# CelestineAngla/BundleAdjustment.jl

Hardware: AMD Instinct MI355X
Metric: LM iterations/sec on BAL venice-1778 (synthetic BAL-shaped), plus Jacobian Mnnz/sec (higher is better)
Workload: dtype f64; 1 GPU; venice-1778 shape: ncams=1778 npnts=993923 nobs=5001946, seed 20261004, lm.jl variant, LDL/None, facto_type f64, fixed 83 iterations, perm AMD; parallelism=points sharded over 1 rank(s), cameras replicated

## Files before the change

### bundleadjustment.jl_amd/csrc/ba_dense_ldl.hip

```cpp
#include "ba_internal.h"

#include <algorithm>
#include <atomic>
#include <cmath>
#include <cstdio>
#include <cstdlib>

namespace {

template <typename T>
struct RT;
template <>
struct RT<double> {
  typedef double v4 __attribute__((ext_vector_type(4)));
  typedef double v2 __attribute__((ext_vector_type(2)));
  static __device__ inline v4 mfma(double a, double b, v4 c) { return __builtin_amdgcn_mfma_f64_16x16x4f64(a, b, c, 0, 0, 0); }
  static __device__ inline int row(int lane, int reg) { return (lane >> 4) + 4 * reg; }
};
template <>
struct RT<float> {
  typedef float v4 __attribute__((ext_vector_type(4)));
  typedef float v2 __attribute__((ext_vector_type(2)));
  static __device__ inline v4 mfma(float a, float b, v4 c) { return __builtin_amdgcn_mfma_f32_16x16x4f32(a, b, c, 0, 0, 0); }
  static __device__ inline int row(int lane, int reg) { return 4 * (lane >> 4) + reg; }
// ... 246 lines not shown
#pragma unroll
      for (int i = m + 1; i < 16; i++) sacc[i] += col[i] * y;
      xj[m * XDL + c] = xv;
      Linv_k[(o + m) * NB + o + c] = xv;
      __builtin_amdgcn_sched_barrier(0);
#pragma unroll
      for (int i = m + 2; i < 16; i++) col[i] = nxt[i];
    }
  };
  auto inv_finalize = [&](int I, int J) {
    d4 acc;
#pragma unroll
    for (int g = 0; g < 4; g++) acc[g] = a[(16 * J + fr) * LDA2 + 16 * I + RT<T>::row(lane, g)];
    d4 out = {0, 0, 0, 0};
#pragma unroll
    for (int g = 0; g < 4; g++) out = RT<T>::mfma(xd[(I * 16 + fr) * XDL + RT<T>::row(lane, g)], acc[g], out);
#pragma unroll
    for (int g = 0; g < 4; g++) {
      a[(16 * J + fr) * LDA2 + 16 * I + RT<T>::row(lane, g)] = -out[g];
      Linv_k[(16 * I + RT<T>::row(lane, g)) * NB + 16 * J + fr] = -out[g];
    }
  };
  auto inv_update = [&](int I, int J, int K) {
    d4 acc = {0, 0, 0, 0};
    if (K > J) {
#pragma unroll
      for (int g = 0; g < 4; g++) acc[g] = a[(16 * J + fr) * LDA2 + 16 * I + RT<T>::row(lane, g)];
    }
#pragma unroll
    for (int kk = 0; kk < 4; kk++) {
      const int k = 16 * K + 4 * kk + fk;
      const T af = a[(16 * I + fr) * LDA2 + k] * dinv[k];
      const T *bp = (K == J) ? xd + (J * 16 + fk) * XDL + fr : a + (16 * J + fr) * LDA2 + 16 * K + fk;
      const int bstep = (K == J) ? 4 * XDL : 4;
      acc = RT<T>::mfma(af, bp[kk * bstep], acc);
    }
#pragma unroll
    for (int g = 0; g < 4; g++) a[(16 * J + fr) * LDA2 + 16 * I + RT<T>::row(lane, g)] = acc[g];
  };
  constexpr int NWK = NW - 1;
  auto do_pivots = [&](int jb) {
    if constexpr (sizeof(T) == 8) pivots_mfma(jb);
    else pivots(jb);
  };
  if (wv == 0) do_pivots(0);
  __syncthreads();
  STAMP(1)
  row_solves(0);
  if (wv == 3 && lane < 16) inv16(0);
  __syncthreads();
  STAMP(2)
  if constexpr (NW == 8) {
    constexpr int CAP = 3 * NWK - 1;
    const int u = (wv == 4) ? 6 : (wv < 4 ? wv - 1 : wv - 2);
    const int h = (wv == 2) ? 0 : (wv == 6) ? 1 : (wv == 4) ? 2 : (wv == 5) ? 3 : (wv == 7) ? 4 : -1;
    auto f_task = [&](int s, int t) {
      int ii = 0;
      while ((ii + 1) * (ii + 2) / 2 <= t) ii++;
      const int jj = t - ii * (ii + 1) / 2;
      block_update(s, s + 2 + ii, s + 2 + jj);
    };
    for (int s = 0; s < 7; s++) {
      const int nX = s, nC = 6 - s, nU = s * (7 - s), nF = (6 - s) * (7 - s) / 2;
      const int nfix = nX + nC + nU, nP = nfix + nF < CAP ? nfix + nF : (nfix > CAP ? nfix : CAP);
      unsigned long long c0 = 0;
      if (stamps) c0 = __builtin_amdgcn_s_memtime();
      if (wv == 0) {
        block_update(s, s + 1, s + 1);
        __builtin_amdgcn_fence(__ATOMIC_RELEASE, "wavefront");
        __builtin_amdgcn_wave_barrier();
        __builtin_amdgcn_fence(__ATOMIC_ACQUIRE, "wavefront");
        do_pivots(s + 1);
      } else {
        for (int r = 0; r < 3 + (nfix + NWK - 1) / NWK; r++) {
          const int t = r < 2 ? NWK * r + u : 2 * NWK + (NWK - 1) * (r - 2) + u;
          if ((r >= 2 && u == NWK - 1) || t >= nP) continue;
          if (t < nX) {
            inv_finalize(s, t);
          } else if (t < nX + nC) {
            block_update(s, s + 2 + (t - nX), s + 1);
          } else if (t < nfix) {
            const int e = t - nX - nC;
            inv_update(s + 1 + e % (7 - s), e / (7 - s), s - 1);
          } else {
            f_task(s, t - nfix);
          }
        }
      }
      if (stamps && lane == 0) stamps[6 + s * 8 + wv] = __builtin_amdgcn_s_memtime() - c0;
      __syncthreads();
      STAMP(1)
      if (stamps) c0 = __builtin_amdgcn_s_memtime();
      row_solves(s + 1);
      if (wv == 3 && lane < 16) inv16(s + 1);
      if (h >= 0) {
        const int nA = (s + 1) + (nfix + nF - nP);
        for (int t = h; t < nA; t += 5) {
          if (t <= s) inv_update(s + 1, t, s);
          else f_task(s, nP - nfix + (t - (s + 1)));
        }
      }
      if (stamps && lane == 0) stamps[62 + s * 8 + wv] = __builtin_amdgcn_s_memtime() - c0;
      __syncthreads();
      STAMP(2)
    }
  } else {
    for (int jb = 0; jb < 7; jb++) {
      for (int t = wv; t < 7; t += NW) {
        if (t < 7 - jb) block_update(jb, jb + 1 + t, jb + 1);
        else inv_finalize(jb, t - (7 - jb));
      }
      __syncthreads();
      STAMP(3)
      unsigned long long c0 = 0;
      if (stamps) c0 = __builtin_amdgcn_s_memtime();
      if (wv == 0) {
        do_pivots(jb + 1);
      } else {
        const int mb = 6 - jb, nblk = mb * (mb + 1) / 2, ninv = (7 - jb) * (jb + 1);
        for (int t = wv - 1; t < nblk + ninv; t += NWK) {
          if (t < nblk) {
            int ii = 0;
            while ((ii + 1) * (ii + 2) / 2 <= t) ii++;
            const int jj = t - ii * (ii + 1) / 2;
            block_update(jb, jb + 2 + ii, jb + 2 + jj);
          } else {
            const int e = t - nblk, J = e / (7 - jb), I = jb + 1 + e % (7 - jb);
            inv_update(I, J, jb);
          }
        }
      }
      if (stamps && lane == 0) stamps[6 + jb * 8 + wv] = __builtin_amdgcn_s_memtime() - c0;
      __syncthreads();
      STAMP(1)
      row_solves(jb + 1);
      if (wv == 3 && lane < 16) inv16(jb + 1);
      __syncthreads();
      STAMP(2)
    }
  }
  for (int J = wv; J < 7; J += NW) inv_finalize(7, J);
  if (tid < NB) D_k[tid] = dd[tid];
  STAMP(4)
  if (stamps && tid == 0)
    for (int q = 0; q < 6; q++) stamps[q] = tacc[q];
#undef STAMP
}

template <typename T>
__global__ __launch_bounds__(DIAG_THREADS) void k_ldl_diag(T *__restrict__ Skk, T *__restrict__ Linv_k,
                                                   T *__restrict__ D_k, int *__restrict__ flag,
                                                   unsigned long long *__restrict__ stamps,
                                                   const int *__restrict__ wait_ready, int clear_flag) {
  extern __shared__ __attribute__((aligned(16))) unsigned char smraw[];
  if (clear_flag && threadIdx.x == 0) *flag = 0;
  if (wait_ready && !hoisted_wait(wait_ready, 1, flag)) return;
  diag_tile<T, DIAG_THREADS / 64>(Skk, Linv_k, D_k, flag, stamps, reinterpret_cast<T *>(smraw));
}

template <typename T>
__global__ __launch_bounds__(DIAG_THREADS) void k_ldl_diag2(T *__restrict__ SkkA, T *__restrict__ LinvA, T *__restrict__ DA,
                                                    T *__restrict__ SkkB, T *__restrict__ LinvB, T *__restrict__ DB,
                                                    int *__restrict__ flag) {
  extern __shared__ __attribute__((aligned(16))) unsigned char smraw[];
  const bool second = blockIdx.x == 1;
  diag_tile<T, DIAG_THREADS / 64>(second ? SkkB : SkkA, second ? LinvB : LinvA, second ? DB : DA, flag, (unsigned long long *)nullptr,
                                  reinterpret_cast<T *>(smraw));
}

template <typename T, int NP, bool YACC = false>
__device__ inline void tile_gemm_abt(const T *__restrict__ A0, const T *__restrict__ B0,
                                     const T *__restrict__ A1, const T *__restrict__ B1, T *sA, T *sB,
                                     typename RT<T>::v4 acc[4][4], const T *__restrict__ bk = nullptr, T *yacc = nullptr) {
  BA_VT
  const int tid = threadIdx.x, lane = tid & 63, wv = tid >> 6;
  const int wr = (wv >> 1) * 64, wc = (wv & 1) * 64;
  const int fr = lane & 15, fk = lane >> 4;
  constexpr int NLD = (NB * KC / 2) / 256;
  d2 pa[NLD], pb[NLD];
  constexpr int UPR = KC / 2;
  constexpr int RPS = 256 / UPR;
  const int lrow = tid / UPR, lc2 = tid % UPR;
#pragma unroll
  for (int it = 0; it < NLD; it++) {
    pa[it] = *reinterpret_cast<const d2 *>(A0 + (lrow + RPS * it) * NB + 2 * lc2);
    pb[it] = *reinterpret_cast<const d2 *>(B0 + (lrow + RPS * it) * NB + 2 * lc2);
  }
  constexpr int NCH = NP * (NB / KC);
  for (int ch = 0; ch < NCH; ch++) {
    __syncthreads();
#pragma unroll
    for (int it = 0; it < NLD; it++) {
      *reinterpret_cast<d2 *>(sA + (lrow + RPS * it) * LDK + 2 * lc2) = pa[it];
      *reinterpret_cast<d2 *>(sB + (lrow + RPS * it) * LDK + 2 * lc2) = pb[it];
    }
    __syncthreads();
    const int nx = ch + 1;
    if (nx < NCH) {
      const T *A = (NP == 2 && nx >= NB / KC) ? A1 : A0;
      const T *B = (NP == 2 && nx >= NB / KC) ? B1 : B0;
      const int k0 = (nx & (NB / KC - 1)) * KC;
#pragma unroll
      for (int it = 0; it < NLD; it++) {
        pa[it] = *reinterpret_cast<const d2 *>(A + (lrow + RPS * it) * NB + k0 + 2 * lc2);
        pb[it] = *reinterpret_cast<const d2 *>(B + (lrow + RPS * it) * NB + k0 + 2 * lc2);
      }
    }
    if (YACC) {
      if (tid < NB) {
        T ya = *yacc;
#pragma unroll
        for (int q = 0; q < KC; q++) ya += sB[tid * LDK + q] * bk[ch * KC + q];
        *yacc = ya;
      }
    }
#pragma unroll
    for (int kk = 0; kk < KC / 4; kk++) {
      T af[4], bf[4];
#pragma unroll
      for (int m = 0; m < 4; m++) af[m] = sA[(wr + 16 * m + fr) * LDK + kk * 4 + fk];
#pragma unroll
      for (int n = 0; n < 4; n++) bf[n] = sB[(wc + 16 * n + fr) * LDK + kk * 4 + fk];
#pragma unroll
      for (int m = 0; m < 4; m++)
#pragma unroll
        for (int n = 0; n < 4; n++) acc[m][n] = RT<T>::mfma(af[m], bf[n], acc[m][n]);
    }
  }
}

template <typename T>
struct PV {
  static constexpr int VL = 16 / sizeof(T);
  static constexpr int KC = 128 / sizeof(T);
  static constexpr int LDK = KC + (sizeof(T) == 8 ? 2 : 4);
  typedef T vu __attribute__((ext_vector_type(16 / sizeof(T))));
};
template <typename T>
constexpr size_t gemm_priv_lds_bytes() { return (size_t)4 * 2 * 64 * PV<T>::LDK * sizeof(T); }
constexpr size_t GEMM_PRIV_LDS_ELEMS = gemm_priv_lds_bytes<double>() / sizeof(double);
template <typename T, int NP>
__device__ inline void tile_gemm_abt_priv(const T *__restrict__ A0, const T *__restrict__ B0,
                                          const T *__restrict__ A1, const T *__restrict__ B1, T *lds,
                                          typename RT<T>::v4 acc[4][4], const T *__restrict__ A2 = nullptr,
                                          const T *__restrict__ B2 = nullptr, const T *__restrict__ A3 = nullptr,
                                          const T *__restrict__ B3 = nullptr) {
  typedef typename PV<T>::vu vu;
  constexpr int PKC = PV<T>::KC, PLDK = PV<T>::LDK, VL = PV<T>::VL;
  const int tid = threadIdx.x, lane = tid & 63, wv = (tid >> 6) & 3;
  const int wr = (wv >> 1) * 64, wc = (wv & 1) * 64;
  const int fr = lane & 15, fk = lane >> 4;
  T *sA = lds + wv * (2 * 64 * PLDK), *sB = sA + 64 * PLDK;
  constexpr int UPR = PKC / VL;
  constexpr int RPS = 64 / UPR;
  constexpr int NLD = 64 / RPS;
  const int lrow = lane / UPR, lc = (lane % UPR) * VL;
  vu pa[NLD], pb[NLD];
  const T *Ab = A0 + wr * NB, *Bb = B0 + wc * NB;
#pragma unroll
  for (int it = 0; it < NLD; it++) {
    pa[it] = *reinterpret_cast<const vu *>(Ab + (lrow + RPS * it) * NB + lc);
    pb[it] = *reinterpret_cast<const vu *>(Bb + (lrow + RPS * it) * NB + lc);
  }
  constexpr int NCH = NP * (NB / PKC);
  for (int ch = 0; ch < NCH; ch++) {
    __builtin_amdgcn_wave_barrier();
#pragma unroll
    for (int it = 0; it < NLD; it++) {
      *reinterpret_cast<vu *>(sA + (lrow + RPS * it) * PLDK + lc) = pa[it];
      *reinterpret_cast<vu *>(sB + (lrow + RPS * it) * PLDK + lc) = pb[it];
    }
    __builtin_amdgcn_fence(__ATOMIC_RELEASE, "wavefront");
    __builtin_amdgcn_wave_barrier();
    __builtin_amdgcn_fence(__ATOMIC_ACQUIRE, "wavefront");
    const int nx = ch + 1;
    if (nx < NCH) {
      const int pn = nx / (NB / PKC);
      const T *A = (pn == 0 ? A0 : pn == 1 ? A1 : pn == 2 ? A2 : A3) + wr * NB;
      const T *B = (pn == 0 ? B0 : pn == 1 ? B1 : pn == 2 ? B2 : B3) + wc * NB;
      const int k0 = (nx & (NB / PKC - 1)) * PKC;
#pragma unroll
      for (int it = 0; it < NLD; it++) {
        pa[it] = *reinterpret_cast<const vu *>(A + (lrow + RPS * it) * NB + k0 + lc);
        pb[it] = *reinterpret_cast<const vu *>(B + (lrow + RPS * it) * NB + k0 + lc);
      }
    }
#pragma unroll
    for (int kk = 0; kk < PKC / 4; kk++) {
      T af[4], bf[4];
#pragma unroll
      for (int m = 0; m < 4; m++) af[m] = sA[(16 * m + fr) * PLDK + kk * 4 + fk];
#pragma unroll
      for (int n = 0; n < 4; n++) bf[n] = sB[(16 * n + fr) * PLDK + kk * 4 + fk];
#pragma unroll
      for (int m = 0; m < 4; m++)
#pragma unroll
        for (int n = 0; n < 4; n++) acc[m][n] = RT<T>::mfma(af[m], bf[n], acc[m][n]);
    }
  }
}

constexpr int RS = 32;
constexpr size_t RS_LDS_ELEMS = (size_t)(2 * (RS + NB) * LDK + 5 * NB);

template <typename T, bool YACC>
__device__ inline void tile_gemm_rows(const T *__restrict__ A, const T *__restrict__ B, T *sA, T *sB,
                                      typename RT<T>::v4 acc[2][2], const T *__restrict__ bk, T *yacc) {
  BA_VT
  const int tid = threadIdx.x, lane = tid & 63, wv = tid >> 6;
  const int wc = wv * 32;
  const int fr = lane & 15, fk = lane >> 4;
  constexpr int UPR = KC / 2;
  const int lrow = tid / UPR, lc2 = tid % UPR;
  constexpr int NCH = NB / KC;
  d2 pa[NCH], pb[NCH][4];
#pragma unroll
  for (int ch = 0; ch < NCH; ch++) {
    pa[ch] = *reinterpret_cast<const d2 *>(A + lrow * NB + ch * KC + 2 * lc2);
#pragma unroll
    for (int it = 0; it < 4; it++) pb[ch][it] = *reinterpret_cast<const d2 *>(B + (lrow + 32 * it) * NB + ch * KC + 2 * lc2);
  }
#pragma unroll
  for (int ch = 0; ch < NCH; ch++) {
    T *cA = sA + (ch & 1) * RS * LDK, *cB = sB + (ch & 1) * NB * LDK;
    *reinterpret_cast<d2 *>(cA + lrow * LDK + 2 * lc2) = pa[ch];
#pragma unroll
    for (int it = 0; it < 4; it++) *reinterpret_cast<d2 *>(cB + (lrow + 32 * it) * LDK + 2 * lc2) = pb[ch][it];
    __syncthreads();
    if (YACC) {
      if (tid < NB) {
        T ya = *yacc;
#pragma unroll
        for (int q = 0; q < KC; q++) ya += cB[tid * LDK + q] * bk[ch * KC + q];
        *yacc = ya;
      }
    }
#pragma unroll
    for (int kk = 0; kk < KC / 4; kk++) {
      T af[2], bf[2];
#pragma unroll
      for (int m = 0; m < 2; m++) af[m] = cA[(16 * m + fr) * LDK + kk * 4 + fk];
#pragma unroll
      for (int n = 0; n < 2; n++) bf[n] = cB[(wc + 16 * n + fr) * LDK + kk * 4 + fk];
#pragma unroll
      for (int m = 0; m < 2; m++)
#pragma unroll
        for (int n = 0; n < 2; n++) acc[m][n] = RT<T>::mfma(af[m], bf[n], acc[m][n]);
    }
  }
  __syncthreads();
}

template <typename T, bool FWD>
__device__ __forceinline__ void ldl_trsm_rs_body(T *__restrict__ S, const int64_t *__restrict__ co, const T *__restrict__ Linv_k,
                                        const T *__restrict__ D_k, T *__restrict__ V, int k, T *__restrict__ b, T *__restrict__ y,
                                        const int *__restrict__ rows, const int bid) {
  BA_VT
  extern __shared__ __attribute__((aligned(16))) unsigned char smraw[];
  T *lds = reinterpret_cast<T *>(smraw);
  T *sA = lds, *sB = lds + 2 * RS * LDK, *ysh = lds + 2 * (RS + NB) * LDK, *red = ysh + NB;
  const int i = rows ? rows[bid >> 2] : k + 1 + (bid >> 2), r0 = (bid & 3) * RS;
  T *Sik = S + tix(co, i, k) * NB * NB + r0 * NB;
  T *Vi = V + (int64_t)i * NB * NB + r0 * NB;
  typename RT<T>::v4 acc[2][2];
#pragma unroll
  for (int m = 0; m < 2; m++)
#pragma unroll
    for (int n = 0; n < 2; n++) acc[m][n] = (d4){0, 0, 0, 0};
  T yacc = 0;
  tile_gemm_rows<T, FWD>(Sik, Linv_k, sA, sB, acc, FWD ? b + (int64_t)k * NB : nullptr, &yacc);
  const int tid = threadIdx.x, lane = tid & 63, wv = tid >> 6, wc = wv * 32;
  if (FWD) {
    if (tid < NB) {
      ysh[tid] = yacc;
      if (bid == 0) y[(int64_t)k * NB + tid] = yacc;
    }
    __syncthreads();
  }
  T part[2][4];
#pragma unroll
  for (int m = 0; m < 2; m++)
#pragma unroll
    for (int g = 0; g < 4; g++) part[m][g] = 0;
#pragma unroll
  for (int n = 0; n < 2; n++) {
    const int col = wc + 16 * n + (lane & 15);
    const T inv_d = (T)1 / D_k[col];
    const T wcol = FWD ? ysh[col] * inv_d : 0.0;
#pragma unroll
    for (int m = 0; m < 2; m++)
#pragma unroll
      for (int g = 0; g < 4; g++) {
        const int row = 16 * m + RT<T>::row(lane, g);
        const T xv = acc[m][n][g];
        Vi[row * NB + col] = xv;
        Sik[row * NB + col] = xv * inv_d;
        if (FWD) part[m][g] += xv * wcol;
      }
  }
  if (FWD) {
#pragma unroll
    for (int m = 0; m < 2; m++)
#pragma unroll
      for (int g = 0; g < 4; g++) {
        T v = part[m][g];
        v += __shfl_xor(v, 1, 64);
        v += __shfl_xor(v, 2, 64);
        v += __shfl_xor(v, 4, 64);
        v += __shfl_xor(v, 8, 64);
        if ((lane & 15) == 0) red[wv * RS + 16 * m + RT<T>::row(lane, g)] = v;
      }
    __syncthreads();
    if (tid < RS) b[(int64_t)i * NB + r0 + tid] -= ((red[tid] + red[RS + tid]) + red[2 * RS + tid]) + red[3 * RS + tid];
  }
}

template <typename T, bool FWD>
__global__ __launch_bounds__(256) void k_ldl_trsm_rs(T *__restrict__ S, const int64_t *__restrict__ co, const T *__restrict__ Linv_k,
                                                      const T *__restrict__ D_k, T *__restrict__ V, int k,
                                                      T *__restrict__ b, T *__restrict__ y,
                                                      const int *__restrict__ rows) {
  ldl_trsm_rs_body<T, FWD>(S, co, Linv_k, D_k, V, k, b, y, rows, (int)blockIdx.x);
}

template <typename T>
struct RunPanel {
  const T *Linv_k, *D_k;
  T *V;
  int k;
  const int *rows;
};
template <typename T, bool FWD>
__global__ __launch_bounds__(256) void k_ldl_trsm_rs2(T *__restrict__ S, const int64_t *__restrict__ co, RunPanel<T> a, RunPanel<T> c, int n0,
                                                       T *__restrict__ b, T *__restrict__ y) {
  const bool second = (int)blockIdx.x >= n0;
  ldl_trsm_rs_body<T, FWD>(S, co, second ? c.Linv_k : a.Linv_k, second ? c.D_k : a.D_k, second ? c.V : a.V, second ? c.k : a.k, b, y,
                           second ? c.rows : a.rows, (int)blockIdx.x - (second ? n0 : 0));
}

template <typename T>
__device__ __forceinline__ void ldl_col_rs_body(T *__restrict__ S, const int64_t *__restrict__ co, const T *__restrict__ V0, int k,
                                       const int *__restrict__ rows, const int bid) {
  BA_VT
  extern __shared__ __attribute__((aligned(16))) unsigned char smraw[];
  T *lds = reinterpret_cast<T *>(smraw);
  T *sA = lds, *sB = lds + 2 * RS * LDK;
  const int i = rows ? rows[bid >> 2] : k + 1 + (bid >> 2), r0 = (bid & 3) * RS;
  typename RT<T>::v4 acc[2][2];
#pragma unroll
  for (int m = 0; m < 2; m++)
#pragma unroll
    for (int n = 0; n < 2; n++) acc[m][n] = (d4){0, 0, 0, 0};
  tile_gemm_rows<T, false>(V0 + (int64_t)i * NB * NB + r0 * NB, S + tix(co, k + 1, k) * NB * NB, sA, sB, acc, nullptr, nullptr);
  const int lane = threadIdx.x & 63, wc = (threadIdx.x >> 6) * 32;
  T *Sij = S + tix(co, i, k + 1) * NB * NB + r0 * NB;
#pragma unroll
  for (int n = 0; n < 2; n++) {
    const int col = wc + 16 * n + (lane & 15);
#pragma unroll
    for (int m = 0; m < 2; m++)
#pragma unroll
      for (int g = 0; g < 4; g++) {
        const int row = 16 * m + RT<T>::row(lane, g);
        Sij[row * NB + col] -= acc[m][n][g];
      }
  }
}

template <typename T>
__global__ __launch_bounds__(256) void k_ldl_col_rs(T *__restrict__ S, const int64_t *__restrict__ co, const T *__restrict__ V0, int k,
                                                     const int *__restrict__ rows) {
  ldl_col_rs_body<T>(S, co, V0, k, rows, (int)blockIdx.x);
}
template <typename T>
__global__ __launch_bounds__(256) void k_ldl_col_rs2(T *__restrict__ S, const int64_t *__restrict__ co, RunPanel<T> a, RunPanel<T> c, int n0) {
  const bool second = (int)blockIdx.x >= n0;
  ldl_col_rs_body<T>(S, co, second ? c.V : a.V, second ? c.k : a.k, second ? c.rows : a.rows, (int)blockIdx.x - (second ? n0 : 0));
}

template <typename T>
__device__ __forceinline__ void ldl_update_rs_body(T *__restrict__ S, const int64_t *__restrict__ co, const T *__restrict__ V0,
                                          const T *__restrict__ V1, int k, int base, int nblk, const int *__restrict__ rows,
                                          int lead_len, const int bid) {
  BA_VT
  extern __shared__ __attribute__((aligned(16))) unsigned char smraw[];
  T *lds = reinterpret_cast<T *>(smraw);
  T *sA = lds, *sB = lds + 2 * RS * LDK;
  const int t = bid >> 2, r0 = (bid & 3) * RS;
  if (t >= nblk) return;
  int ii, jj;
  if (lead_len > 0) {
    jj = t < lead_len ? 0 : 1;
    ii = t < lead_len ? t : t - lead_len + 1;
  } else {
    ii = (int)((sqrt(8.0 * (double)t + 1.0) - 1.0) * 0.5);
    while ((ii + 1) * (ii + 2) / 2 <= t) ii++;
    while (ii * (ii + 1) / 2 > t) ii--;
    jj = t - ii * (ii + 1) / 2;
  }
  const int i = rows ? rows[ii] : base + ii, j = rows ? rows[jj] : base + jj;
  typename RT<T>::v4 acc[2][2];
#pragma unroll
  for (int m = 0; m < 2; m++)
#pragma unroll
    for (int n = 0; n < 2; n++) acc[m][n] = (d4){0, 0, 0, 0};
  tile_gemm_rows<T, false>(V0 + (int64_t)i * NB * NB + r0 * NB, S + tix(co, j, k) * NB * NB, sA, sB, acc, nullptr, nullptr);
  tile_gemm_rows<T, false>(V1 + (int64_t)i * NB * NB + r0 * NB, S + tix(co, j, k + 1) * NB * NB, sA, sB, acc, nullptr, nullptr);
  const int lane = threadIdx.x & 63, wc = (threadIdx.x >> 6) * 32;
  T *Sij = S + tix(co, i, j) * NB * NB + r0 * NB;
#pragma unroll
  for (int n = 0; n < 2; n++) {
    const int col = wc + 16 * n + (lane & 15);
#pragma unroll
    for (int m = 0; m < 2; m++)
#pragma unroll
      for (int g = 0; g < 4; g++) {
        const int row = 16 * m + RT<T>::row(lane, g);
        Sij[row * NB + col] -= acc[m][n][g];
      }
  }
}

template <typename T>
__global__ __launch_bounds__(256) void k_ldl_update_rs(T *__restrict__ S, const int64_t *__restrict__ co, const T *__restrict__ V0,
                                                        const T *__restrict__ V1, int k, int base, int nblk,
                                                        const int *__restrict__ rows, int lead_len) {
  ldl_update_rs_body<T>(S, co, V0, V1, k, base, nblk, rows, lead_len, (int)blockIdx.x);
}
template <typename T>
__global__ __launch_bounds__(256) void k_ldl_update_rs2(T *__restrict__ S, const int64_t *__restrict__ co, RunPanel<T> a, int nblk_a,
                                                         RunPanel<T> c, int nblk_c, int64_t panel, int lead_a, int lead_c) {
  const bool second = (int)blockIdx.x >= 4 * nblk_a;
  const RunPanel<T> &r = second ? c : a;
  ldl_update_rs_body<T>(S, co, r.V, r.V + panel, r.k, r.k + 2, second ? nblk_c : nblk_a, r.rows, second ? lead_c : lead_a,
                        (int)blockIdx.x - (second ? 4 * nblk_a : 0));
}

constexpr int LDX = NB + 4;
constexpr size_t PT_LDS_ELEMS = (size_t)(RS * LDX + 2 * NB * LDK + 2 * NB + 4 * RS);

template <typename T>
__device__ inline void tile_gemm_rows_ldsA(const T *sX, const T *__restrict__ B, T *sB, typename RT<T>::v4 acc[2][2]) {
  BA_VT
  const int tid = threadIdx.x, lane = tid & 63, wv = tid >> 6;
  const int wc = wv * 32;
  const int fr = lane & 15, fk = lane >> 4;
  constexpr int UPR = KC / 2;
  const int lrow = tid / UPR, lc2 = tid % UPR;
  constexpr int NCH = NB / KC;
  d2 pb[NCH][4];
#pragma unroll
  for (int ch = 0; ch < NCH; ch++)
#pragma unroll
    for (int it = 0; it < 4; it++) pb[ch][it] = *reinterpret_cast<const d2 *>(B + (lrow + 32 * it) * NB + ch * KC + 2 * lc2);
#pragma unroll
  for (int ch = 0; ch < NCH; ch++) {
    T *cB = sB + (ch & 1) * NB * LDK;
#pragma unroll
    for (int it = 0; it < 4; it++) *reinterpret_cast<d2 *>(cB + (lrow + 32 * it) * LDK + 2 * lc2) = pb[ch][it];
    __syncthreads();
#pragma unroll
    for (int kk = 0; kk < KC / 4; kk++) {
      T af[2], bf[2];
#pragma unroll
      for (int m = 0; m < 2; m++) af[m] = sX[(16 * m + fr) * LDX + ch * KC + kk * 4 + fk];
#pragma unroll
      for (int n = 0; n < 2; n++) bf[n] = cB[(wc + 16 * n + fr) * LDK + kk * 4 + fk];
#pragma unroll
      for (int m = 0; m < 2; m++)
#pragma unroll
        for (int n = 0; n < 2; n++) acc[m][n] = RT<T>::mfma(af[m], bf[n], acc[m][n]);
    }
  }
  __syncthreads();
}

template <typename T, bool FWD>
__global__ __launch_bounds__(256) void k_ldl_pairtrsm(T *__restrict__ S, const int64_t *__restrict__ co, const T *__restrict__ Linv,
                                                       const T *__restrict__ D, T *__restrict__ V0, T *__restrict__ V1, int k,
                                                       T *__restrict__ b, const T *__restrict__ y) {
  BA_VT
  extern __shared__ __attribute__((aligned(16))) unsigned char smraw[];
  T *lds = reinterpret_cast<T *>(smraw);
  T *sX = lds, *sB = sX + RS * LDX, *ysh = sB + 2 * NB * LDK, *red = ysh + 2 * NB;
  const int i = k + 2 + (blockIdx.x >> 2), r0 = (blockIdx.x & 3) * RS;
  const int tid = threadIdx.x, lane = tid & 63, wv = tid >> 6, wc = wv * 32;
  T *Sik = S + tix(co, i, k) * NB * NB + r0 * NB;
  T *Sik1 = S + tix(co, i, k + 1) * NB * NB + r0 * NB;
  T *Vi0 = V0 + (int64_t)i * NB * NB + r0 * NB, *Vi1 = V1 + (int64_t)i * NB * NB + r0 * NB;
  const T *Dk = D + (int64_t)k * NB, *Dk1 = Dk + NB;
  if (FWD) ysh[tid] = y[(int64_t)k * NB + tid];
  typename RT<T>::v4 acc[2][2];
  T part[2][4];
#pragma unroll
  for (int m = 0; m < 2; m++)
#pragma unroll
    for (int g = 0; g < 4; g++) part[m][g] = 0;
#pragma unroll
  for (int m = 0; m < 2; m++)
#pragma unroll
    for (int n = 0; n < 2; n++) acc[m][n] = (d4){0, 0, 0, 0};
  {
    d2 v[8];
#pragma unroll
    for (int q = 0; q < 8; q++) v[q] = *reinterpret_cast<const d2 *>(Sik + 2 * (q * 256 + tid));
#pragma unroll
    for (int q = 0; q < 8; q++) {
      const int idx = 2 * (q * 256 + tid);
      *reinterpret_cast<d2 *>(sX + (idx >> 7) * LDX + (idx & (NB - 1))) = v[q];
    }
  }
  tile_gemm_rows_ldsA<T>(sX, Linv + (int64_t)k * NB * NB, sB, acc);
#pragma unroll
  for (int n = 0; n < 2; n++) {
    const int col = wc + 16 * n + (lane & 15);
    const T inv_d = (T)1 / Dk[col];
    const T wcol = FWD ? ysh[col] * inv_d : (T)0;
#pragma unroll
    for (int m = 0; m < 2; m++)
#pragma unroll
      for (int g = 0; g < 4; g++) {
        const int row = 16 * m + RT<T>::row(lane, g);
        const T xv = acc[m][n][g];
        Vi0[row * NB + col] = xv;
        Sik[row * NB + col] = xv * inv_d;
        sX[row * LDX + col] = xv;
        if (FWD) part[m][g] += xv * wcol;
      }
  }
#pragma unroll
  for (int m = 0; m < 2; m++)
#pragma unroll
    for (int n = 0; n < 2; n++) acc[m][n] = (d4){0, 0, 0, 0};
  tile_gemm_rows_ldsA<T>(sX, S + tix(co, k + 1, k) * NB * NB, sB, acc);
#pragma unroll
  for (int n = 0; n < 2; n++) {
    const int col = wc + 16 * n + (lane & 15);
#pragma unroll
    for (int m = 0; m < 2; m++)
#pragma unroll
      for (int g = 0; g < 4; g++) {
        const int row = 16 * m + RT<T>::row(lane, g);
        sX[row * LDX + col] = Sik1[row * NB + col] - acc[m][n][g];
      }
  }
#pragma unroll
  for (int m = 0; m < 2; m++)
#pragma unroll
    for (int n = 0; n < 2; n++) acc[m][n] = (d4){0, 0, 0, 0};
  tile_gemm_rows_ldsA<T>(sX, Linv + (int64_t)(k + 1) * NB * NB, sB, acc);
#pragma unroll
  for (int n = 0; n < 2; n++) {
    const int col = wc + 16 * n + (lane & 15);
    const T inv_d = (T)1 / Dk1[col];
    const T wcol = FWD ? ysh[NB + col] * inv_d : (T)0;
#pragma unroll
    for (int m = 0; m < 2; m++)
#pragma unroll
      for (int g = 0; g < 4; g++) {
        const int row = 16 * m + RT<T>::row(lane, g);
        const T xv = acc[m][n][g];
        Vi1[row * NB + col] = xv;
        Sik1[row * NB + col] = xv * inv_d;
        if (FWD) part[m][g] += xv * wcol;
      }
  }
  if (FWD) {
#pragma unroll
    for (int m = 0; m < 2; m++)
#pragma unroll
      for (int g = 0; g < 4; g++) {
        T v = part[m][g];
        v += __shfl_xor(v, 1, 64);
        v += __shfl_xor(v, 2, 64);
        v += __shfl_xor(v, 4, 64);
        v += __shfl_xor(v, 8, 64);
        if ((lane & 15) == 0) red[wv * RS + 16 * m + RT<T>::row(lane, g)] = v;
      }
    __syncthreads();
    if (tid < RS) b[(int64_t)i * NB + r0 + tid] -= ((red[tid] + red[RS + tid]) + red[2 * RS + tid]) + red[3 * RS + tid];
  }
}

template <typename T, bool FWD>
__global__ __launch_bounds__(256) void k_ldl_pairdiag(T *__restrict__ S, const int64_t *__restrict__ co, T *__restrict__ Linv,
                                                       T *__restrict__ D, T *__restrict__ V0, int k, int nt,
                                                       int *__restrict__ flag, const int *__restrict__ wait_ready, int need,
                                                       T *__restrict__ b, T *__restrict__ y) {
  BA_VT
  extern __shared__ __attribute__((aligned(16))) unsigned char smraw[];
  T *sm = reinterpret_cast<T *>(smraw);
  if (wait_ready && !hoisted_wait(wait_ready, need, flag)) return;
  const int tid = threadIdx.x, lane = tid & 63, wv = tid >> 6;
  T *Skk = S + tix(co, k, k) * NB * NB, *Lk = Linv + (int64_t)k * NB * NB, *Dk = D + (int64_t)k * NB;
  diag_tile<T, 4>(Skk, Lk, Dk, flag, nullptr, sm);
  __threadfence();
  __syncthreads();
  T *ysh = sm + 2 * NB * LDK;
  if (FWD) {
    if (tid < NB) {
      T sacc = 0;
      for (int c = 0; c <= tid; c++) sacc += Lk[tid * NB + c] * b[(int64_t)k * NB + c];
      ysh[tid] = sacc;
      y[(int64_t)k * NB + tid] = sacc;
    }
    __syncthreads();
  }
  if (k + 1 >= nt) return;
  T *S10 = S + tix(co, k + 1, k) * NB * NB, *S11 = S + tix(co, k + 1, k + 1) * NB * NB;
  T *V10 = V0 + (int64_t)(k + 1) * NB * NB;
  const int wr = (wv >> 1) * 64, wc = (wv & 1) * 64;
  typename RT<T>::v4 acc[4][4];
#pragma unroll
  for (int m = 0; m < 4; m++)
#pragma unroll
    for (int n = 0; n < 4; n++) acc[m][n] = (d4){0, 0, 0, 0};
  tile_gemm_abt<T, 1>(S10, Lk, nullptr, nullptr, sm, sm + NB * LDK, acc);
#pragma unroll
  for (int n = 0; n < 4; n++) {
    const int col = wc + 16 * n + (lane & 15);
    const T inv_d = (T)1 / Dk[col];
#pragma unroll
    for (int m = 0; m < 4; m++)
#pragma unroll
      for (int g = 0; g < 4; g++) {
        const int row = wr + 16 * m + RT<T>::row(lane, g);
        const T xv = acc[m][n][g];
        V10[row * NB + col] = xv;
        S10[row * NB + col] = xv * inv_d;
      }
  }
  __threadfence();
  __syncthreads();
  if (FWD) {
    if (tid < NB) {
      T sacc = 0;
      for (int c = 0; c < NB; c++) sacc += S10[tid * NB + c] * ysh[c];
      b[(int64_t)(k + 1) * NB + tid] -= sacc;
    }
  }
#pragma unroll
  for (int m = 0; m < 4; m++)
#pragma unroll
    for (int n = 0; n < 4; n++) acc[m][n] = (d4){0, 0, 0, 0};
  tile_gemm_abt<T, 1>(V10, S10, nullptr, nullptr, sm, sm + NB * LDK, acc);
#pragma unroll
  for (int n = 0; n < 4; n++) {
    const int col = wc + 16 * n + (lane & 15);
#pragma unroll
    for (int m = 0; m < 4; m++)
#pragma unroll
      for (int g = 0; g < 4; g++) {
        const int row = wr + 16 * m + RT<T>::row(lane, g);
        S11[row * NB + col] -= acc[m][n][g];
      }
  }
  __threadfence();
  __syncthreads();
  T *Lk1 = Lk + NB * NB, *Dk1 = Dk + NB;
  diag_tile<T, 4>(S11, Lk1, Dk1, flag, nullptr, sm);
  if (FWD) {
    __threadfence();
    __syncthreads();
    if (tid < NB) {
      T sacc = 0;
      for (int c = 0; c <= tid; c++) sacc += Lk1[tid * NB + c] * b[(int64_t)(k + 1) * NB + c];
      y[(int64_t)(k + 1) * NB + tid] = sacc;
    }
  }
}

template <typename T>
__device__ __forceinline__ int ldl_update_tile(T *__restrict__ S, const int64_t *__restrict__ co, const T *__restrict__ V0, const T *__restrict__ V1,
                                      int k, int i, int j, T *lds, const T *__restrict__ Lp0, const T *__restrict__ Lp1,
                                      int *__restrict__ ticket = nullptr) {
  BA_VT
  T *Sij = S + tix(co, i, j) * NB * NB;
  typename RT<T>::v4 acc[4][4];
#pragma unroll
  for (int m = 0; m < 4; m++)
#pragma unroll
    for (int n = 0; n < 4; n++) acc[m][n] = (d4){0, 0, 0, 0};
  tile_gemm_abt_priv<T, 2>(V0 + (int64_t)i * NB * NB, Lp0 ? Lp0 + (int64_t)j * NB * NB : S + tix(co, j, k) * NB * NB,
                        V1 + (int64_t)i * NB * NB, Lp1 ? Lp1 + (int64_t)j * NB * NB : S + tix(co, j, k + 1) * NB * NB, lds, acc);
  int tid2 = threadIdx.x;
  asm volatile("" : "+v"(tid2));
  int drawn = 0;
  if (ticket && tid2 == 0) drawn = __hip_atomic_fetch_add(ticket, 1, __ATOMIC_RELAXED, __HIP_MEMORY_SCOPE_AGENT);
  const int lane = tid2 & 63, wv = (tid2 >> 6) & 3;
  const int wr = (wv >> 1) * 64, wc = (wv & 1) * 64;
  T *cbase = Sij + wr * NB + wc + (lane & 15);
#pragma unroll
  for (int h = 0; h < 2; h++) {
    T cv[2][4][4];
#pragma unroll
    for (int n2 = 0; n2 < 2; n2++)
#pragma unroll
      for (int m = 0; m < 4; m++)
#pragma unroll
        for (int g = 0; g < 4; g++) cv[n2][m][g] = cbase[(16 * m + RT<T>::row(lane, g)) * NB + 16 * (2 * h + n2)];
#pragma unroll
    for (int n2 = 0; n2 < 2; n2++)
#pragma unroll
      for (int m = 0; m < 4; m++)
#pragma unroll
        for (int g = 0; g < 4; g++) {
          const T nv = cv[n2][m][g] - acc[m][2 * h + n2][g];
          cbase[(16 * m + RT<T>::row(lane, g)) * NB + 16 * (2 * h + n2)] = nv;
        }
  }
  return drawn;
}

template <typename T, int MODE, bool OWN = false>
__global__ __launch_bounds__(256, 2) void k_ldl_update(T *__restrict__ S, const int64_t *__restrict__ co, const T *__restrict__ V0,
                                                        const T *__restrict__ V1, int k, int base, int nt, int nblk,
                                                        int *__restrict__ ready, const int *__restrict__ own_cols,
                                                        const int64_t *__restrict__ own_pref, int m0, int m_end, int ready_tiles,
                                                        const int *__restrict__ rows, const T *__restrict__ Lp0,
                                                        const T *__restrict__ Lp1, const int2 *__restrict__ tlist, int blocked,
                                                        int *__restrict__ tickets) {
  BA_VT
  static_assert(MODE == 1, "only the pair update is a tile-per-workgroup kernel");
  extern __shared__ __attribute__((aligned(16))) unsigned char smraw[];
  T *lds = reinterpret_cast<T *>(smraw);
  if constexpr (!OWN) {
    if (tickets) {
      __shared__ int s_next[2], s_src[2];
      int m_rows = (int)((sqrt(8.0 * (double)nblk + 1.0) - 1.0) * 0.5);
      while ((m_rows + 1) * (m_rows + 2) / 2 <= nblk) m_rows++;
      while (m_rows * (m_rows + 1) / 2 > nblk) m_rows--;
      const int nready = ready ? ready_tiles : 0;
      const int xcd = (int)(__builtin_amdgcn_s_getreg(20 | (0 << 6) | ((4 - 1) << 11)) & (TICKET_QUEUES - 1));
      const bool wave0 = __builtin_amdgcn_readfirstlane((int)(threadIdx.x >> 6)) == 0;
      auto take = [&](int src, int drawn, int slot) {
        const bool first = (threadIdx.x & 63) == 0;
        int n_raw = __builtin_amdgcn_readfirstlane(drawn), t;
        for (;;) {
          t = ticket_tile(nblk, nready, ticket_source(xcd, src), n_raw);
          if (t >= 0 || src == TICKET_QUEUES) break;
          src++;
          int v = 0;
          if (first) v = __hip_atomic_fetch_add(tickets + ticket_source(xcd, src), 1, __ATOMIC_RELAXED, __HIP_MEMORY_SCOPE_AGENT);
          n_raw = __builtin_amdgcn_readfirstlane(v);
        }
        if (first) {
          s_next[slot] = t;
          s_src[slot] = src;
        }
      };
      if (wave0) {
        int v = 0;
        if (threadIdx.x == 0) v = __hip_atomic_fetch_add(tickets + TICKET_READY, 1, __ATOMIC_RELAXED, __HIP_MEMORY_SCOPE_AGENT);
        take(0, v, 0);
      }
      const int sb = blocked > 0 ? blocked : TSB;
      for (int par = 0;; par ^= 1) {
        __syncthreads();
        const int t = __builtin_amdgcn_readfirstlane(s_next[par]);
        if (t < 0) return;
        const int src = __builtin_amdgcn_readfirstlane(s_src[par]);
        int ii, jj;
        tri_blocked(t, m_rows, &ii, &jj, sb);
        const int n_raw = ldl_update_tile<T>(S, co, V0, V1, k, rows ? rows[ii] : base + ii, rows ? rows[jj] : base + jj, lds, Lp0, Lp1,
                                             tickets + ticket_source(xcd, src));
        if (ready && t < ready_tiles) {
          __threadfence();
          __syncthreads();
          if (threadIdx.x == 0) __hip_atomic_fetch_add(ready, 1, __ATOMIC_RELEASE, __HIP_MEMORY_SCOPE_AGENT);
        }
        if (wave0) take(src, n_raw, par ^ 1);
      }
    }
  }
  int i, j, tsel;
  {
    const int per = (nblk + 7) / 8;
    int t = (blockIdx.x & 7) * per + (blockIdx.x >> 3);
    if (t >= nblk) return;
    tsel = t;
    if (tlist) {
      i = tlist[t].x;
      j = tlist[t].y;
    } else if (OWN) {
      const int64_t tt = t + own_pref[m0];
      int lo = m0, hi = m_end;
      while (hi - lo > 1) {
        const int mid = (lo + hi) >> 1;
        if (own_pref[mid] <= tt) lo = mid;
        else hi = mid;
      }
      j = own_cols[lo];
      i = j + (int)(tt - own_pref[lo]);
    } else {
      int m_rows = (int)((sqrt(8.0 * (double)nblk + 1.0) - 1.0) * 0.5);
      while ((m_rows + 1) * (m_rows + 2) / 2 <= nblk) m_rows++;
      while (m_rows * (m_rows + 1) / 2 > nblk) m_rows--;
      int ii, jj;
      if (blocked) {
        tri_blocked(t, m_rows, &ii, &jj, blocked);
      } else {
        ii = (int)((sqrt(8.0 * (double)t + 1.0) - 1.0) * 0.5);
        while ((ii + 1) * (ii + 2) / 2 <= t) ii++;
        while (ii * (ii + 1) / 2 > t) ii--;
        jj = t - ii * (ii + 1) / 2;
      }
      i = rows ? rows[ii] : base + ii;
      j = rows ? rows[jj] : base + jj;
    }
  }
  ldl_update_tile<T>(S, co, V0, V1, k, i, j, lds, Lp0, Lp1);
  if (ready && tsel < ready_tiles) {
    __threadfence();
    __syncthreads();
    if (threadIdx.x == 0) __hip_atomic_fetch_add(ready, 1, __ATOMIC_RELEASE, __HIP_MEMORY_SCOPE_AGENT);
  }
}

template <typename T>
constexpr size_t part_lds_bytes() { return 2 * gemm_priv_lds_bytes<T>(); }
template <typename T>
__global__ __launch_bounds__(512) void k_ldl_update_part(T *__restrict__ S, const int64_t *__restrict__ co, const T *__restrict__ V0,
                                                          const T *__restrict__ V1, int k, int nblk, const int *__restrict__ rows,
                                                          int base) {
  extern __shared__ __attribute__((aligned(16))) unsigned char smraw[];
  const int half = __builtin_amdgcn_readfirstlane((int)(threadIdx.x >> 8));
  T *lds = reinterpret_cast<T *>(smraw + half * gemm_priv_lds_bytes<T>());
  for (int t = 2 * blockIdx.x + half; t < nblk; t += 2 * gridDim.x) {
    int ii = (int)((sqrt(8.0 * (double)t + 1.0) - 1.0) * 0.5);
    while ((ii + 1) * (ii + 2) / 2 <= t) ii++;
    while (ii * (ii + 1) / 2 > t) ii--;
    const int jj = t - ii * (ii + 1) / 2;
    ldl_update_tile<T>(S, co, V0, V1, k, rows ? rows[ii] : base + ii, rows ? rows[jj] : base + jj, lds, nullptr, nullptr);
  }
}

template <typename T>
__global__ __launch_bounds__(512) void k_ldl_update_part2(T *__restrict__ S, const int64_t *__restrict__ co, RunPanel<T> a, int nblk_a,
                                                           RunPanel<T> c, int nblk_c, int64_t panel) {
  extern __shared__ __attribute__((aligned(16))) unsigned char smraw[];
  const int half = __builtin_amdgcn_readfirstlane((int)(threadIdx.x >> 8));
  T *lds = reinterpret_cast<T *>(smraw + half * gemm_priv_lds_bytes<T>());
  for (int tt = 2 * blockIdx.x + half; tt < nblk_a + nblk_c; tt += 2 * gridDim.x) {
    const bool second = tt >= nblk_a;
    const RunPanel<T> &r = second ? c : a;
    const int t = tt - (second ? nblk_a : 0);
    int ii = (int)((sqrt(8.0 * (double)t + 1.0) - 1.0) * 0.5);
    while ((ii + 1) * (ii + 2) / 2 <= t) ii++;
    while (ii * (ii + 1) / 2 > t) ii--;
    const int jj = t - ii * (ii + 1) / 2;
    ldl_update_tile<T>(S, co, r.V, r.V + panel, r.k, r.rows[ii], r.rows[jj], lds, nullptr, nullptr);
  }
}

template <typename T>
__global__ __launch_bounds__(256, 2) void k_ldl_update2(T *__restrict__ S, const int64_t *__restrict__ co, RunPanel<T> a, int nblk_a,
                                                         RunPanel<T> c, int nblk_c, int64_t panel) {
  extern __shared__ __attribute__((aligned(16))) unsigned char smraw[];
  T *lds = reinterpret_cast<T *>(smraw);
  const int ga = ((nblk_a + 7) / 8) * 8;
  const bool second = (int)blockIdx.x >= ga;
  const RunPanel<T> &r = second ? c : a;
  const int nblk = second ? nblk_c : nblk_a, bid = (int)blockIdx.x - (second ? ga : 0);
  const int per = (nblk + 7) / 8;
  const int t = (bid & 7) * per + (bid >> 3);
  if (t >= nblk) return;
  int ii = (int)((sqrt(8.0 * (double)t + 1.0) - 1.0) * 0.5);
  while ((ii + 1) * (ii + 2) / 2 <= t) ii++;
  while (ii * (ii + 1) / 2 > t) ii--;
  const int jj = t - ii * (ii + 1) / 2;
// ... 1090 lines not shown
```

Before: 28.35 LM iterations/s.

## Exploit triangular Linv in row-panel TRSM and prefetch operands ahead in pair TRSM

Treats the inverse diagonal factor Linv as lower triangular, so the row-panel GEMMs load only the nonzero 16x16 block columns per chunk and skip MFMAs on the zero blocks. Work is balanced across waves by pairing block column wv with 7-wv. Because of that column permutation, the forward-solve dot product is moved into a separate LDS-staged pass. The pair TRSM kernel also prefetches the next GEMM's B operand, the D values and the Sik1 tile into registers during earlier chunks, and sets a 2-blocks-per-SM launch bound. Risks include extra register pressure, the added LDS round-trip and sync, and reliance on Linv being exactly triangular.

```diff
diff --git a/bundleadjustment.jl_amd/csrc/ba_dense_ldl.hip b/bundleadjustment.jl_amd/csrc/ba_dense_ldl.hip
--- a/bundleadjustment.jl_amd/csrc/ba_dense_ldl.hip
+++ b/bundleadjustment.jl_amd/csrc/ba_dense_ldl.hip
@@ -572,51 +572,98 @@
 
 constexpr int RS = 32;
 constexpr size_t RS_LDS_ELEMS = (size_t)(2 * (RS + NB) * LDK + 5 * NB);
-
-template <typename T, bool YACC>
+constexpr int LDX = NB + 4;
+static_assert(RS * LDX <= 2 * (RS + NB) * LDK, "the panel solve puts its 32 x 128 result where the chunk ring was");
+
+constexpr int NCHR = NB / KC;
+static_assert(KC == 16 && NCHR == 8, "the triangular products take one 16 x 16 block column of the inverse per chunk");
+template <typename T>
+struct BRows {
+  typename RT<T>::v2 v[NCHR][4];
+};
+template <bool TRI>
+__host__ __device__ constexpr int brows_pieces(int ch) { return TRI ? (NCHR - ch + 1) / 2 : 4; }
+template <bool TRI>
+__device__ __forceinline__ bool brows_held(int ch, int it, int lrow) {
+  return !TRI || (NCHR - ch) % 2 == 0 || it + 1 < brows_pieces<TRI>(ch) || lrow < 16;
+}
+template <typename T, bool TRI, int C0 = 0, int C1 = NCHR>
+__device__ __forceinline__ void brows_request(const T *__restrict__ B, BRows<T> &pb) {
+  typedef typename RT<T>::v2 d2;
+  const int lrow = threadIdx.x / (KC / 2), lc2 = threadIdx.x % (KC / 2);
+#pragma unroll
+  for (int ch = C0; ch < C1; ch++)
+#pragma unroll
+    for (int it = 0; it < 4; it++)
+      if (it < brows_pieces<TRI>(ch) && brows_held<TRI>(ch, it, lrow))
+        pb.v[ch][it] = *reinterpret_cast<const d2 *>(B + ((TRI ? KC * ch : 0) + lrow + 32 * it) * NB + ch * KC + 2 * lc2);
+}
+template <typename T, bool TRI>
+__device__ __forceinline__ void brows_stage(const BRows<T> &pb, int ch, T *cB) {
+  typedef typename RT<T>::v2 d2;
+  const int lrow = threadIdx.x / (KC / 2), lc2 = threadIdx.x % (KC / 2);
+#pragma unroll
+  for (int it = 0; it < 4; it++)
+    if (it < brows_pieces<TRI>(ch) && brows_held<TRI>(ch, it, lrow))
+      *reinterpret_cast<d2 *>(cB + ((TRI ? KC * ch : 0) + lrow + 32 * it) * LDK + 2 * lc2) = pb.v[ch][it];
+}
+template <bool TRI>
+__device__ __forceinline__ int rs_cblock(int wv, int n) { return TRI ? (n == 0 ? wv : NCHR - 1 - wv) : 2 * wv + n; }
+
+template <typename T, bool N0>
+__device__ __forceinline__ void rows_chunk_mma(const T *cA, int lda, const T *cB, int cb0, int cb1, typename RT<T>::v4 acc[2][2]) {
+  const int lane = threadIdx.x & 63, fr = lane & 15, fk = lane >> 4;
+#pragma unroll
+  for (int kk = 0; kk < KC / 4; kk++) {
+    T af[2], bf[2];
+#pragma unroll
+    for (int m = 0; m < 2; m++) af[m] = cA[(16 * m + fr) * lda + kk * 4 + fk];
+    if (N0) bf[0] = cB[(16 * cb0 + fr) * LDK + kk * 4 + fk];
+    bf[1] = cB[(16 * cb1 + fr) * LDK + kk * 4 + fk];
+#pragma unroll
+    for (int m = 0; m < 2; m++) {
+      if (N0) acc[m][0] = RT<T>::mfma(af[m], bf[0], acc[m][0]);
+      acc[m][1] = RT<T>::mfma(af[m], bf[1], acc[m][1]);
+    }
+  }
+}
+template <typename T, bool TRI>
+__device__ __forceinline__ void rows_chunk(const T *cA, int lda, const T *cB, int ch, typename RT<T>::v4 acc[2][2]) {
+  const int wv = __builtin_amdgcn_readfirstlane(threadIdx.x >> 6);
+  const int cb0 = rs_cblock<TRI>(wv, 0), cb1 = rs_cblock<TRI>(wv, 1);
+  if (!TRI || (ch < NCHR / 2 && ch <= cb0))
+    rows_chunk_mma<T, true>(cA, lda, cB, cb0, cb1, acc);
+  else if (ch <= cb1)
+    rows_chunk_mma<T, false>(cA, lda, cB, cb0, cb1, acc);
+}
+
+template <typename T, bool YACC, bool TRI = false>
 __device__ inline void tile_gemm_rows(const T *__restrict__ A, const T *__restrict__ B, T *sA, T *sB,
                                       typename RT<T>::v4 acc[2][2], const T *__restrict__ bk, T *yacc) {
   BA_VT
-  const int tid = threadIdx.x, lane = tid & 63, wv = tid >> 6;
-  const int wc = wv * 32;
-  const int fr = lane & 15, fk = lane >> 4;
+  const int tid = threadIdx.x;
   constexpr int UPR = KC / 2;
   const int lrow = tid / UPR, lc2 = tid % UPR;
-  constexpr int NCH = NB / KC;
-  d2 pa[NCH], pb[NCH][4];
-#pragma unroll
-  for (int ch = 0; ch < NCH; ch++) {
-    pa[ch] = *reinterpret_cast<const d2 *>(A + lrow * NB + ch * KC + 2 * lc2);
-#pragma unroll
-    for (int it = 0; it < 4; it++) pb[ch][it] = *reinterpret_cast<const d2 *>(B + (lrow + 32 * it) * NB + ch * KC + 2 * lc2);
-  }
-#pragma unroll
-  for (int ch = 0; ch < NCH; ch++) {
+  d2 pa[NCHR];
+  BRows<T> pb;
+#pragma unroll
+  for (int ch = 0; ch < NCHR; ch++) pa[ch] = *reinterpret_cast<const d2 *>(A + lrow * NB + ch * KC + 2 * lc2);
+  brows_request<T, TRI>(B, pb);
+#pragma unroll
+  for (int ch = 0; ch < NCHR; ch++) {
     T *cA = sA + (ch & 1) * RS * LDK, *cB = sB + (ch & 1) * NB * LDK;
     *reinterpret_cast<d2 *>(cA + lrow * LDK + 2 * lc2) = pa[ch];
-#pragma unroll
-    for (int it = 0; it < 4; it++) *reinterpret_cast<d2 *>(cB + (lrow + 32 * it) * LDK + 2 * lc2) = pb[ch][it];
+    brows_stage<T, TRI>(pb, ch, cB);
     __syncthreads();
     if (YACC) {
-      if (tid < NB) {
+      if (tid < NB && (!TRI || tid >= KC * ch)) {
         T ya = *yacc;
 #pragma unroll
         for (int q = 0; q < KC; q++) ya += cB[tid * LDK + q] * bk[ch * KC + q];
         *yacc = ya;
       }
     }
-#pragma unroll
-    for (int kk = 0; kk < KC / 4; kk++) {
-      T af[2], bf[2];
-#pragma unroll
-      for (int m = 0; m < 2; m++) af[m] = cA[(16 * m + fr) * LDK + kk * 4 + fk];
-#pragma unroll
-      for (int n = 0; n < 2; n++) bf[n] = cB[(wc + 16 * n + fr) * LDK + kk * 4 + fk];
-#pragma unroll
-      for (int m = 0; m < 2; m++)
-#pragma unroll
-        for (int n = 0; n < 2; n++) acc[m][n] = RT<T>::mfma(af[m], bf[n], acc[m][n]);
-    }
+    rows_chunk<T, TRI>(cA, LDK, cB, ch, acc);
   }
   __syncthreads();
 }
@@ -638,25 +685,21 @@
 #pragma unroll
     for (int n = 0; n < 2; n++) acc[m][n] = (d4){0, 0, 0, 0};
   T yacc = 0;
-  tile_gemm_rows<T, FWD>(Sik, Linv_k, sA, sB, acc, FWD ? b + (int64_t)k * NB : nullptr, &yacc);
   const int tid = threadIdx.x, lane = tid & 63, wv = tid >> 6, wc = wv * 32;
-  if (FWD) {
-    if (tid < NB) {
-      ysh[tid] = yacc;
-      if (bid == 0) y[(int64_t)k * NB + tid] = yacc;
-    }
-    __syncthreads();
-  }
-  T part[2][4];
-#pragma unroll
-  for (int m = 0; m < 2; m++)
-#pragma unroll
-    for (int g = 0; g < 4; g++) part[m][g] = 0;
+  T dcol[2];
+#pragma unroll
+  for (int n = 0; n < 2; n++) dcol[n] = D_k[16 * rs_cblock<true>(wv, n) + (lane & 15)];
+  const T dy = FWD && tid < NB ? D_k[tid] : (T)1;
+  tile_gemm_rows<T, FWD, true>(Sik, Linv_k, sA, sB, acc, FWD ? b + (int64_t)k * NB : nullptr, &yacc);
+  T *sXf = lds;
+  if (FWD && tid < NB) {
+    ysh[tid] = yacc * ((T)1 / dy);
+    if (bid == 0) y[(int64_t)k * NB + tid] = yacc;
+  }
 #pragma unroll
   for (int n = 0; n < 2; n++) {
-    const int col = wc + 16 * n + (lane & 15);
-    const T inv_d = (T)1 / D_k[col];
-    const T wcol = FWD ? ysh[col] * inv_d : 0.0;
+    const int col = 16 * rs_cblock<true>(wv, n) + (lane & 15);
+    const T inv_d = (T)1 / dcol[n];
 #pragma unroll
     for (int m = 0; m < 2; m++)
 #pragma unroll
@@ -665,10 +708,25 @@
         const T xv = acc[m][n][g];
         Vi[row * NB + col] = xv;
         Sik[row * NB + col] = xv * inv_d;
-        if (FWD) part[m][g] += xv * wcol;
+        if (FWD) sXf[row * LDX + col] = xv;
       }
   }
   if (FWD) {
+    __syncthreads();
+    T part[2][4];
+#pragma unroll
+    for (int m = 0; m < 2; m++)
+#pragma unroll
+      for (int g = 0; g < 4; g++) part[m][g] = 0;
+#pragma unroll
+    for (int n = 0; n < 2; n++) {
+      const int col = wc + 16 * n + (lane & 15);
+      const T wcol = ysh[col];
+#pragma unroll
+      for (int m = 0; m < 2; m++)
+#pragma unroll
+        for (int g = 0; g < 4; g++) part[m][g] += sXf[(16 * m + RT<T>::row(lane, g)) * LDX + col] * wcol;
+    }
 #pragma unroll
     for (int m = 0; m < 2; m++)
 #pragma unroll
@@ -806,86 +864,86 @@
                         (int)blockIdx.x - (second ? 4 * nblk_a : 0));
 }
 
-constexpr int LDX = NB + 4;
 constexpr size_t PT_LDS_ELEMS = (size_t)(RS * LDX + 2 * NB * LDK + 2 * NB + 4 * RS);
-
-template <typename T>
-__device__ inline void tile_gemm_rows_ldsA(const T *sX, const T *__restrict__ B, T *sB, typename RT<T>::v4 acc[2][2]) {
-  BA_VT
-  const int tid = threadIdx.x, lane = tid & 63, wv = tid >> 6;
-  const int wc = wv * 32;
-  const int fr = lane & 15, fk = lane >> 4;
-  constexpr int UPR = KC / 2;
-  const int lrow = tid / UPR, lc2 = tid % UPR;
-  constexpr int NCH = NB / KC;
-  d2 pb[NCH][4];
-#pragma unroll
-  for (int ch = 0; ch < NCH; ch++)
-#pragma unroll
-    for (int it = 0; it < 4; it++) pb[ch][it] = *reinterpret_cast<const d2 *>(B + (lrow + 32 * it) * NB + ch * KC + 2 * lc2);
-#pragma unroll
-  for (int ch = 0; ch < NCH; ch++) {
+constexpr int PT_AHEAD1 = 4, PT_AHEAD2 = 7;
+template <typename T, bool TRI, typename F>
+__device__ __forceinline__ void tile_gemm_rows_ldsA(const T *sX, const BRows<T> &pb, T *sB, typename RT<T>::v4 acc[2][2], F ahead) {
+#pragma unroll
+  for (int ch = 0; ch < NCHR; ch++) {
     T *cB = sB + (ch & 1) * NB * LDK;
-#pragma unroll
-    for (int it = 0; it < 4; it++) *reinterpret_cast<d2 *>(cB + (lrow + 32 * it) * LDK + 2 * lc2) = pb[ch][it];
+    brows_stage<T, TRI>(pb, ch, cB);
     __syncthreads();
-#pragma unroll
-    for (int kk = 0; kk < KC / 4; kk++) {
-      T af[2], bf[2];
-#pragma unroll
-      for (int m = 0; m < 2; m++) af[m] = sX[(16 * m + fr) * LDX + ch * KC + kk * 4 + fk];
-#pragma unroll
-      for (int n = 0; n < 2; n++) bf[n] = cB[(wc + 16 * n + fr) * LDK + kk * 4 + fk];
-#pragma unroll
-      for (int m = 0; m < 2; m++)
-#pragma unroll
-        for (int n = 0; n < 2; n++) acc[m][n] = RT<T>::mfma(af[m], bf[n], acc[m][n]);
-    }
+    ahead(ch);
+    rows_chunk<T, TRI>(sX + ch * KC, LDX, cB, ch, acc);
   }
   __syncthreads();
 }
 
 template <typename T, bool FWD>
-__global__ __launch_bounds__(256) void k_ldl_pairtrsm(T *__restrict__ S, const int64_t *__restrict__ co, const T *__restrict__ Linv,
-                                                       const T *__restrict__ D, T *__restrict__ V0, T *__restrict__ V1, int k,
-                                                       T *__restrict__ b, const T *__restrict__ y) {
+__global__ __launch_bounds__(256, 2) void k_ldl_pairtrsm(T *__restrict__ S, const int64_t *__restrict__ co, const T *__restrict__ Linv,
+                                                          const T *__restrict__ D, T *__restrict__ V0, T *__restrict__ V1, int k,
+                                                          T *__restrict__ b, const T *__restrict__ y) {
   BA_VT
   extern __shared__ __attribute__((aligned(16))) unsigned char smraw[];
   T *lds = reinterpret_cast<T *>(smraw);
   T *sX = lds, *sB = sX + RS * LDX, *ysh = sB + 2 * NB * LDK, *red = ysh + 2 * NB;
   const int i = k + 2 + (blockIdx.x >> 2), r0 = (blockIdx.x & 3) * RS;
-  const int tid = threadIdx.x, lane = tid & 63, wv = tid >> 6, wc = wv * 32;
+  const int tid = threadIdx.x, lane = tid & 63, wv = tid >> 6, wc = wv * 32, fr = lane & 15;
   T *Sik = S + tix(co, i, k) * NB * NB + r0 * NB;
   T *Sik1 = S + tix(co, i, k + 1) * NB * NB + r0 * NB;
   T *Vi0 = V0 + (int64_t)i * NB * NB + r0 * NB, *Vi1 = V1 + (int64_t)i * NB * NB + r0 * NB;
   const T *Dk = D + (int64_t)k * NB, *Dk1 = Dk + NB;
-  if (FWD) ysh[tid] = y[(int64_t)k * NB + tid];
+  const T *Linv_k = Linv + (int64_t)k * NB * NB, *Linv_k1 = Linv_k + NB * NB, *L10 = S + tix(co, k + 1, k) * NB * NB;
+  T yv = 0, dv = 1;
+  if (FWD) {
+    yv = y[(int64_t)k * NB + tid];
+    dv = Dk[tid];
+  }
+  d2 v[8];
+#pragma unroll
+  for (int q = 0; q < 8; q++) v[q] = *reinterpret_cast<const d2 *>(Sik + 2 * (q * 256 + tid));
+  BRows<T> pb1, pb2, pb3;
+  brows_request<T, true>(Linv_k, pb1);
+  T dcol[2][2];
+  T c1[2][2][4];
+  if (FWD) ysh[tid] = yv * ((T)1 / dv);
   typename RT<T>::v4 acc[2][2];
   T part[2][4];
 #pragma unroll
   for (int m = 0; m < 2; m++)
 #pragma unroll
     for (int g = 0; g < 4; g++) part[m][g] = 0;
+  auto fwd_part = [&](const T *w) {
+#pragma unroll
+    for (int n = 0; n < 2; n++) {
+      const int col = wc + 16 * n + fr;
+      const T wcol = w[col];
+#pragma unroll
+      for (int m = 0; m < 2; m++)
+#pragma unroll
+        for (int g = 0; g < 4; g++) part[m][g] += sX[(16 * m + RT<T>::row(lane, g)) * LDX + col] * wcol;
+    }
+  };
 #pragma unroll
   for (int m = 0; m < 2; m++)
 #pragma unroll
     for (int n = 0; n < 2; n++) acc[m][n] = (d4){0, 0, 0, 0};
-  {
-    d2 v[8];
-#pragma unroll
-    for (int q = 0; q < 8; q++) v[q] = *reinterpret_cast<const d2 *>(Sik + 2 * (q * 256 + tid));
-#pragma unroll
-    for (int q = 0; q < 8; q++) {
-      const int idx = 2 * (q * 256 + tid);
-      *reinterpret_cast<d2 *>(sX + (idx >> 7) * LDX + (idx & (NB - 1))) = v[q];
-    }
-  }
-  tile_gemm_rows_ldsA<T>(sX, Linv + (int64_t)k * NB * NB, sB, acc);
+#pragma unroll
+  for (int q = 0; q < 8; q++) {
+    const int idx = 2 * (q * 256 + tid);
+    *reinterpret_cast<d2 *>(sX + (idx >> 7) * LDX + (idx & (NB - 1))) = v[q];
+  }
+  tile_gemm_rows_ldsA<T, true>(sX, pb1, sB, acc, [&](int ch) {
+    if (ch == PT_AHEAD1) {
+#pragma unroll
+      for (int n = 0; n < 2; n++) dcol[0][n] = Dk[16 * rs_cblock<true>(wv, n) + fr];
+      brows_request<T, false, 0, NCHR / 2>(L10, pb2);
+    }
+  });
 #pragma unroll
   for (int n = 0; n < 2; n++) {
-    const int col = wc + 16 * n + (lane & 15);
-    const T inv_d = (T)1 / Dk[col];
-    const T wcol = FWD ? ysh[col] * inv_d : (T)0;
+    const int col = 16 * rs_cblock<true>(wv, n) + fr;
+    const T inv_d = (T)1 / dcol[0][n];
 #pragma unroll
     for (int m = 0; m < 2; m++)
 #pragma unroll
@@ -895,35 +953,46 @@
         Vi0[row * NB + col] = xv;
         Sik[row * NB + col] = xv * inv_d;
         sX[row * LDX + col] = xv;
-        if (FWD) part[m][g] += xv * wcol;
       }
   }
 #pragma unroll
   for (int m = 0; m < 2; m++)
 #pragma unroll
     for (int n = 0; n < 2; n++) acc[m][n] = (d4){0, 0, 0, 0};
-  tile_gemm_rows_ldsA<T>(sX, S + tix(co, k + 1, k) * NB * NB, sB, acc);
+  tile_gemm_rows_ldsA<T, false>(sX, pb2, sB, acc, [&](int ch) {
+    if (ch == 0) {
+      brows_request<T, false, NCHR / 2, NCHR>(L10, pb2);
+#pragma unroll
+      for (int n = 0; n < 2; n++)
+#pragma unroll
+        for (int m = 0; m < 2; m++)
+#pragma unroll
+          for (int g = 0; g < 4; g++) c1[n][m][g] = Sik1[(16 * m + RT<T>::row(lane, g)) * NB + wc + 16 * n + fr];
+    }
+    if (ch == PT_AHEAD2) {
+      brows_request<T, true>(Linv_k1, pb3);
+#pragma unroll
+      for (int n = 0; n < 2; n++) dcol[1][n] = Dk1[16 * rs_cblock<true>(wv, n) + fr];
+    }
+    if (FWD && ch == NCHR - 1) fwd_part(ysh);
+  });
 #pragma unroll
   for (int n = 0; n < 2; n++) {
-    const int col = wc + 16 * n + (lane & 15);
+    const int col = wc + 16 * n + fr;
 #pragma unroll
     for (int m = 0; m < 2; m++)
 #pragma unroll
-      for (int g = 0; g < 4; g++) {
-        const int row = 16 * m + RT<T>::row(lane, g);
-        sX[row * LDX + col] = Sik1[row * NB + col] - acc[m][n][g];
-      }
+      for (int g = 0; g < 4; g++) sX[(16 * m + RT<T>::row(lane, g)) * LDX + col] = c1[n][m][g] - acc[m][n][g];
   }
 #pragma unroll
   for (int m = 0; m < 2; m++)
 #pragma unroll
     for (int n = 0; n < 2; n++) acc[m][n] = (d4){0, 0, 0, 0};
-  tile_gemm_rows_ldsA<T>(sX, Linv + (int64_t)(k + 1) * NB * NB, sB, acc);
+  tile_gemm_rows_ldsA<T, true>(sX, pb3, sB, acc, [](int) {});
 #pragma unroll
   for (int n = 0; n < 2; n++) {
-    const int col = wc + 16 * n + (lane & 15);
-    const T inv_d = (T)1 / Dk1[col];
-    const T wcol = FWD ? ysh[NB + col] * inv_d : (T)0;
+    const int col = 16 * rs_cblock<true>(wv, n) + fr;
+    const T inv_d = (T)1 / dcol[1][n];
 #pragma unroll
     for (int m = 0; m < 2; m++)
 #pragma unroll
@@ -932,10 +1001,12 @@
         const T xv = acc[m][n][g];
         Vi1[row * NB + col] = xv;
         Sik1[row * NB + col] = xv * inv_d;
-        if (FWD) part[m][g] += xv * wcol;
+        if (FWD) sX[row * LDX + col] = xv;
       }
   }
   if (FWD) {
+    __syncthreads();
+    fwd_part(ysh + NB);
 #pragma unroll
     for (int m = 0; m < 2; m++)
 #pragma unroll
```

After: 28.46 LM iterations/s, median of 6. No clear change (+0.4%).
